# qcc4cp/qcc

Hardware: AMD Instinct MI355X
Metric: gate-applies/sec (2^30-amplitude units), QFT (higher is better)
Workload: dtype f64; 1 GPU; 30-qubit QFT complex128, 465 gates/step (qc.qft order), basis-state input, state resident in HBM, 2^30 amplitudes per GPU [BASELINE config 2]; qubits=30, fusion=1

## Files before the change

### include/qcc_hip.h

```cpp
#ifndef QCC_HIP_H_
#define QCC_HIP_H_

#include <stdint.h>

#ifdef __cplusplus
extern "C" {
#endif

typedef struct qh_state_s *qh_handle;

#define QH_OK 0
#define QH_ERR_BAD_QUBIT 1
#define QH_ERR_SAME_QUBIT 2
#define QH_ERR_BAD_DTYPE 3
#define QH_ERR_HIP 4
#define QH_ERR_ARG 5
#define QH_ERR_NOMEM 6
#define QH_ERR_NO_DEVICE 7
#define QH_ERR_NONLOCAL 8
#define QH_ERR_COMM 9

#define QH_FUSE_OFF 0
#define QH_FUSE_SWEEP 1

// ... 77 lines not shown
int qh_comm_unique_id(void *id );
int qh_comm_init(qh_handle h, int nranks, int rank, const void *id);
int qh_comm_init_custom(qh_handle h, int nranks, int rank, qh_round_fn fn, void *user);
int qh_comm_destroy(qh_handle h);
int qh_exchange_alltoall(qh_handle h, int base_bit, uint64_t chunk_amps);
int qh_exchange_pair(qh_handle h, int shard_bit, int local_bit, uint64_t chunk_amps);
int qh_exchange_loopback(qh_handle h, int local_bit, uint64_t chunk_amps);
int qh_exchange_wait(qh_handle h);
int qh_exchange_stats(qh_handle h, qh_xstats *out);
int qh_comm_allreduce_sum(qh_handle h, double *inout, int count);

int qh_norm2(qh_handle h, double *out);
int qh_amplitude(qh_handle h, uint64_t logical_index, double out[2]);
int qh_argmax(qh_handle h, uint64_t *phys_index, double *prob);
int qh_prob_bit(qh_handle h, int logical_bit, double *p1);
int qh_prob_bit_value(qh_handle h, int logical_bit, int value, double *p);
int qh_scale(qh_handle h, double re, double im);
int qh_project_bit(qh_handle h, int logical_bit, int value);
int qh_marginal(qh_handle h, int k, const int32_t *bits, double *out);
int qh_sample(qh_handle h, uint64_t count, const double *u, uint64_t *logical_out);
int qh_project_bits(qh_handle h, uint64_t mask, uint64_t value);
int qh_expect_pauli(qh_handle h, uint64_t nterms, const uint64_t *xmask, const uint64_t *zmask, double *out);

typedef struct {
  uint64_t gates_submitted;
  uint64_t kernels_launched;
  uint64_t sweeps;
  uint64_t bytes_algorithmic;
  uint64_t bytes_swept;
  uint64_t gates_noop;
} qh_stats;
int qh_get_stats(qh_handle h, qh_stats *out);
int qh_reset_stats(qh_handle h);
int qh_timer_begin(qh_handle h);
int qh_timer_end(qh_handle h, float *milliseconds);
int qh_timer_lap(qh_handle h);
int qh_timer_laps(qh_handle h, float *milliseconds, int cap, int *count);
int qh_plan_json(qh_handle h, char *buf, uint64_t cap, uint64_t *needed);

int qh_plan_export(qh_handle h, void *buf, uint64_t cap, uint64_t *needed);

int qh_plan_handlers(qh_handle h, void *buf, uint64_t cap, uint64_t *needed);

int qh_host_apply1(void *psi, const double gate[8], int nbits, int tgt,
                   int bit_width);
int qh_host_applyc(void *psi, const double gate[8], int nbits, int ctl, int tgt,
                   int bit_width);
int qh_host_release(void);

#ifdef __cplusplus
}
#endif
#endif
```

### qcc_amd/csrc/engine.hip

```cpp
#include <hip/hip_runtime.h>

#include <algorithm>
#include <chrono>
#include <cmath>
#include <cstdarg>
#include <cstddef>
#include <cstdio>
#include <cstdlib>
#include <cstring>
#include <ctime>
#include <string>
#include <vector>

#include "../../include/qcc_hip.h"
#include "kernels_gate.hip.h"
#include "kernels_dense.hip.h"
#include "kernels_mux.hip.h"
#include "kernels_measure.hip.h"
#include "kernels_expect.hip.h"
#include "planner.h"
#include "kernels_sweep.hip.h"

namespace {

// ... 306 lines not shown
        abort_comm_and_drain(h);
        return fail(QH_ERR_COMM, "%s: rank %d of %d still waiting after %.0f s (QH_COMM_TIMEOUT_MS): a peer is missing or the "
                    "ranks disagree about an exchange; the communicator was aborted, the state of this handle is undefined", what,
                    h->comm->rank, h->comm->nranks, ms * 1e-3);
      }
      struct timespec ts = {0, 50000};
      nanosleep(&ts, nullptr);
    }
  }
}
int wait_stream(qh_state_s *h, hipStream_t s, const char *what) {
  if (!watched(h)) {
    HIP_TRY(hipStreamSynchronize(s));
    return QH_OK;
  }
  return poll_until_done(h, [&] { return hipStreamQuery(s); }, what);
}
int wait_event(qh_state_s *h, hipEvent_t e, const char *what) {
  if (!watched(h)) {
    HIP_TRY(hipEventSynchronize(e));
    return QH_OK;
  }
  return poll_until_done(h, [&] { return hipEventQuery(e); }, what);
}

bool relayout_eligible(const qh_state_s *h) {
  return env_int("QH_RELAYOUT", 1) != 0 && h->owns_mem && !h->host_psi && qh::sweep_supported(h->nloc, h->bw);
}
bool relayout_wanted(const qh_state_s *h) {
  if (h->dry) return env_int("QH_RELAYOUT", 1) != 0;
  if (h->relayout >= 0) return h->relayout == 1;
  return relayout_eligible(h) && !(h->comm && h->comm->nranks > 1);
}
qh::PlanRequest plan_request(const qh_state_s *h, bool relayout) {
  return qh::PlanRequest{h->nloc, h->bw, h->shard, relayout, h->nglob > h->nloc, qh::PlanSwitches::from_env()};
}
hipError_t alloc_state_buffer(void **p, size_t bytes) {
  static const int contig = env_int("QH_ALLOC_CONTIG", -1), debug = env_int("QH_ALLOC_DEBUG", 0);
  const auto t0 = std::chrono::steady_clock::now();
  hipError_t e = hipErrorOutOfMemory;
  bool got_contig = false;
  const bool want_contig = contig < 0 ? (bytes >= (4ull << 30) && bytes <= (32ull << 30)) : (contig > 0 && bytes >= (64ull << 20));
  if (want_contig) {
    e = hipExtMallocWithFlags(p, bytes, hipDeviceMallocContiguous);
    got_contig = e == hipSuccess;
    if (!got_contig) {
      (void)hipGetLastError();
      *p = nullptr;
    }
  }
  if (!got_contig) e = hipMalloc(p, bytes);
  if (debug)
    fprintf(stderr, "[qh alloc %zu MiB %s at %p in %.1f ms]\n", bytes >> 20, got_contig ? "contiguous" : "plain", *p,
            std::chrono::duration<double, std::milli>(std::chrono::steady_clock::now() - t0).count());
  return e;
}
bool second_buffer_fits(const qh_state_s *h, size_t bytes) {
  size_t fr = 0, total = 0;
  const size_t reserve = (bytes >> 5) + (3ull << 29) + ((h->comm && h->comm->nranks > 1) ? (4ull << 30) : 0);
  return hipMemGetInfo(&fr, &total) == hipSuccess && fr > bytes + reserve;
}
bool alloc_second_buffer(qh_state_s *h) {
  if (h->d_alt) return true;
  const size_t bytes = (size_t)h->amp_bytes() << h->nloc;
  if (second_buffer_fits(h, bytes) && alloc_state_buffer(&h->d_alt, bytes) == hipSuccess)
    return true;
  (void)hipGetLastError();
  h->d_alt = nullptr;
// ... 46 lines not shown
  }
  if (borrowed) {
    if (rc) (void)hipStreamSynchronize(h->stream);
    (void)hipFree(h->d_alt);
    h->d_alt = nullptr;
  } else if (rc == QH_OK) {
    std::swap(h->d_psi, h->d_alt);
  }
  if (rc) return rc;
  for (size_t k = 0; k < loc.size(); ++k) h->perm[loc[k]] = posn[k];
  return QH_OK;
}

int flush_impl(qh_state_s *h, qh::SlabIO *split = nullptr, qh::TileMaxOut *tmax = nullptr) {
  int rc = use_device(h);
  if (rc) return rc;
  if (h->poisoned)
    return fail(QH_ERR_HIP, "the state of this handle is undefined: a sweep of an earlier flush failed after others had run; "
                            "re-initialise it (qh_init_basis / qh_init_product / qh_upload of the whole shard)");
  std::vector<qh::Arrival> *arr = (h->comm && !h->comm->arrivals.empty()) ? &h->comm->arrivals : nullptr;
  if (h->queue.empty()) {
    qh::wait_all_arrivals(arr, h->stream);
    return QH_OK;
  }
  if (h->fusion == QH_FUSE_SWEEP && qh::sweep_supported(h->nloc, h->bw)) {
    const uint64_t launched0 = h->stats.kernels_launched;
    qh::SlabIO local;
    qh::SlabIO *io = split ? split : &local;
    io->arrivals = arr;
    io->comm = h->comm;
    const bool relay = relayout_ready(h);
    void *result = h->d_psi;
    uint8_t final_pos[64];
    rc = qh::run_fused(h->queue, plan_request(h, relay), h->d_psi, h->stream, h->dry, &h->sweep, &h->stats, &g_err,
                       h->comm ? io : nullptr, h->d_alt, &result, final_pos, tmax);
    if (rc == QH_OK && relay) {
      if (result != h->d_psi) std::swap(h->d_psi, h->d_alt);
      for (int b = 0; b < h->nglob; ++b)
        if (h->perm[b] < h->nloc) h->perm[b] = final_pos[h->perm[b]];
    }
    qh::wait_all_arrivals(arr, h->stream);
    if (h->comm) h->comm->stats.sweeps_overlapped += io->sweeps_overlapped;
    if (rc != QH_OK && h->stats.kernels_launched == launched0) return rc;
    if (rc == QH_OK) rc = check_launch(h);
    if (rc != QH_OK) {
      g_err += " [sweeps of this flush may have run partially: its gates were dropped and the state is undefined until re-initialised]";
      h->poisoned = true;
    }
    h->queue.clear();
    return rc;
  }
  qh::wait_all_arrivals(arr, h->stream);
  size_t done = 0;
  for (const auto &r : h->queue) {
    rc = launch_single(h, r);
    if (rc == QH_OK) rc = check_launch(h);
    if (rc) break;
    ++done;
  }
  h->queue.erase(h->queue.begin(), h->queue.begin() + done);
  return rc;
}

int enter(qh_state_s *h) {
  if (h->dry) return fail(QH_ERR_ARG, "not on a dry (planner-only) handle");
  return flush_impl(h);
}
// ... 1352 lines not shown
      for (uint32_t u = 0; u < (1u << per_bits); ++u) a.zu[k] |= (uint16_t)((__builtin_popcount(u & zu) & 1) << u);
      a.zc[k] = z >> nom;
      const uint32_t one = (((tm.ny >> 1) ^ tm.neg) & 1u) ? 0xBFF00000u : 0x3FF00000u;
      if (tm.ny & 1u) a.cim[k] = one; else a.cre[k] = one;
    }
    const int tt = cnt <= 4 ? 4 : qh::kExpectT;
    with_real(h, [&](auto x) {
      using R = decltype(x);
      if (tt == 4) launch_expect<R, 4>(h, pair, (unsigned)nblk, a, slab);
      else launch_expect<R, qh::kExpectT>(h, pair, (unsigned)nblk, a, slab);
    });
    hipLaunchKernelGGL(qh::k_expect_fold, dim3((unsigned)cnt), dim3(256), 0, h->stream, (const double *)slab, (uint32_t)nblk, tt,
                       pair ? 2.0 : 1.0, dout + first);
    if ((rc = check_launch(h))) return rc;
    first += cnt;
    ++batches;
  }
  std::vector<double> vals(nterms);
  if ((rc = read_back(h, vals.data(), dout, (size_t)nterms * sizeof(double)))) return rc;
  for (uint64_t k = 0; k < nterms; ++k) out[terms[k].idx] = vals[k];
  h->stats.kernels_launched += batches;
  h->stats.bytes_swept += batches * ((1ull << h->nloc) * h->amp_bytes());
  return QH_OK;
}

int qh_get_stats(qh_handle h, qh_stats *out) {
  if (!h || !out) return fail(QH_ERR_ARG, "null");
  *out = h->stats;
  return QH_OK;
}
int qh_reset_stats(qh_handle h) {
  if (!h) return fail(QH_ERR_ARG, "null");
  h->stats = qh_stats{};
  return QH_OK;
}

int qh_timer_begin(qh_handle h) {
  if (!h) return fail(QH_ERR_ARG, "null handle");
  int rc = enter(h);
  if (rc) return rc;
  rc = make_events(h);
  if (rc) return rc;
  HIP_TRY(hipEventRecord(h->ev0, h->stream));
  return QH_OK;
}
int qh_timer_end(qh_handle h, float *ms) {
  if (!h || !ms) return fail(QH_ERR_ARG, "null handle or out");
  if (!h->ev0) return fail(QH_ERR_ARG, "qh_timer_end without qh_timer_begin");
  int rc = enter(h);
  if (rc) return rc;
  HIP_TRY(hipEventRecord(h->ev1, h->stream));
  if ((rc = wait_event(h, h->ev1, "qh_timer_end"))) return rc;
  HIP_TRY(hipEventElapsedTime(ms, h->ev0, h->ev1));
  return QH_OK;
}

int qh_timer_lap(qh_handle h) {
  if (!h) return fail(QH_ERR_ARG, "null handle");
  const int rc = enter(h);
  if (rc) return rc;
  if (h->laps_used == h->laps.size()) {
    hipEvent_t e = nullptr;
    HIP_TRY(hipEventCreate(&e));
    h->laps.push_back(e);
  }
  HIP_TRY(hipEventRecord(h->laps[h->laps_used++], h->stream));
// ... 718 lines not shown
```

### qcc_amd/csrc/kernels_sweep.hip.h

```cpp
#pragma once
#include <hip/hip_runtime.h>

#include <string>
#include <vector>

#include "kernels_gate.hip.h"
#include <deque>
#include <memory>

#include "planner.h"
#include "exchange.hip.h"

namespace qh {

struct SweepParams {
  const SweepOp *ops;
  const DGroup *groups;
  const OTerm *oterms;
  uint32_t nops;
  uint32_t tables_rel;
  uint32_t n_ltab_lds;
  uint32_t pad0;
  uint64_t store_delta_mask;
  uint64_t prof_buf;
// ... 292 lines not shown
      memcpy(&o->cm_reg, &g.re, 8);
      memcpy(&o->cm_thread, &g.im, 8);
    }
  if (!sp.groups.empty()) memcpy(groups_out, sp.groups.data(), sp.groups.size() * sizeof(DGroup));
  for (size_t k = 0; k < sp.groups.size(); ++k) {
    DGroup *g = groups_out + k;
    if (n_ltab_lds && (g->flags & DG_LTAB) && g->ltab_off / 64 < n_ltab_lds) g->flags |= DG_LTAB_LDS;
    bool sign_ot = !(g->flags & (DG_LTAB | DG_BITFAC)) && g->ntab == 0 && g->n_oterms > 0 && g->re == 1.0 && g->im == 0.0;
    for (uint32_t t = 0; sign_ot && t < g->n_oterms; ++t) {
      const OTerm &o = sp.oterms[g->oterm_off + t];
      sign_ot = o.re == -1.0 && o.im == 0.0;
    }
    g->flags |= group_handler_bits(*g, sp.rb, sign_ot);
  }
}

struct PlanCacheEntry {
  std::vector<GateRec> queue;
  std::string key;
  std::shared_ptr<const PlanResult> plan;
};

inline bool same_queue(const std::vector<GateRec> &a, const std::vector<GateRec> &b) {
  if (a.size() != b.size()) return false;
  for (size_t i = 0; i < a.size(); ++i)
    if (a[i].ctl_mask != b[i].ctl_mask || a[i].tgt != b[i].tgt || a[i].neg_mask != b[i].neg_mask ||
        memcmp(a[i].g, b[i].g, sizeof a[i].g) != 0)
      return false;
  return true;
}

struct SweepBuffers {
  std::deque<PlanCacheEntry> plans;
  void *d_buf = nullptr;
  size_t cap = 0;
  void *h_pinned = nullptr;
  size_t cap_host = 0;
  hipEvent_t copied = nullptr;
};

inline void free_sweep_buffers(SweepBuffers *b) {
  if (b->copied) {
    (void)hipEventSynchronize(b->copied);
    (void)hipEventDestroy(b->copied);
  }
  if (b->d_buf) (void)hipFree(b->d_buf);
  if (b->h_pinned) (void)hipHostFree(b->h_pinned);
  *b = SweepBuffers{};
}

inline bool sweep_supported(int nloc, int bw) { return (bw == 128 || bw == 64) && nloc >= kLaneBits + 2; }

template <bool WIDE> inline void sweep_block_shape(const SweepPlan &sp, int *wpb, size_t *exch_bytes) {
  const bool contiguous = sp.contiguous();
  *wpb = contiguous ? 2 : 4;
  *exch_bytes = 0;
  if (sp.nwave) {
    *wpb = 1 << sp.nwave;
    const int nr = 1 << sp.rb;
    *exch_bytes = (size_t)*wpb * std::min(8, nr / 2) * 64 * (WIDE ? 16 : 8);
  }
}

template <bool WIDE> inline int ltab_lds_count(const SweepPlan &sp) {
  constexpr int cap = 16;
  int wpb;
  size_t exch;
  sweep_block_shape<WIDE>(sp, &wpb, &exch);
  const long per_wg = 160l * 1024 * wpb / 12 - (long)exch - 512;
  const int fit = (int)std::max(0l, per_wg / 1024);
  return std::max(0, std::min(std::min(sp.n_ltab, cap), fit));
}

inline int sweep_rot(bool contiguous) { return contiguous ? 3 : 6; }

inline uint64_t sweep_tile_bits(const SweepPlan &sp) {
  uint64_t m = ((1ull << sp.lane_low) - 1) | sp.fixed_ones;
  for (int k = 0; k < sp.rb; ++k) m |= (1ull << sp.regpos[k]) | (1ull << sp.regpos_store[k]);
  for (int k = 0; k < sp.nlanehi(); ++k) m |= 1ull << sp.lanehi[k];
  for (int k = 0; k < sp.nwave; ++k) m |= 1ull << sp.wavepos[k];
  return m;
// ... 120 lines not shown
  uint64_t tile_mask = 0;
};

struct SlabIO {
  std::vector<Arrival> *arrivals = nullptr;
  bool split_last = false;
  uint64_t avoid = 0;
  int want_bits = 3;
  Comm *comm = nullptr;
  uint64_t slab_mask = 0;
  std::vector<uint64_t> slab_vals;
  std::vector<hipEvent_t> slab_done;
  bool split_done = false;
  uint64_t sweeps_overlapped = 0;
};

inline void wait_all_arrivals(std::vector<Arrival> *arr, hipStream_t stream) {
  if (!arr) return;
  for (const Arrival &a : *arr) if (a.ev) (void)hipStreamWaitEvent(stream, a.ev, 0);
  arr->clear();
}

inline int run_fused(const std::vector<GateRec> &queue, const PlanRequest &rq, void *psi, hipStream_t stream, bool dry,
                     SweepBuffers *bufs, qh_stats *stats, std::string *err, SlabIO *slab = nullptr, void *psi_alt = nullptr,
                     void **result = nullptr, uint8_t *final_pos = nullptr, TileMaxOut *tmax = nullptr) {
  const int nloc = rq.nloc, bw = rq.bw;
  const uint64_t shard = rq.shard;
  std::shared_ptr<const PlanResult> cached;
  const int rc = guard_planning(err, [&] {
    const std::string key = rq.key();
    const bool use_cache = !getenv("QH_PLAN_CACHE") || atoi(getenv("QH_PLAN_CACHE")) != 0;
    if (use_cache)
      for (auto &e : bufs->plans)
        if (e.key == key && same_queue(e.queue, queue)) { cached = e.plan; return; }
    cached = std::make_shared<const PlanResult>(plan_best(queue, rq));
    if (use_cache) {
      bufs->plans.push_front(PlanCacheEntry{queue, key, cached});
      if (bufs->plans.size() > 4) bufs->plans.pop_back();
    }
  });
  if (rc) return rc;
  const PlanResult &pr = *cached;
  const int pace = dry ? 0 : flush_pace(pr, bw == 128, nloc);
  stats->gates_noop += pr.noop_gates;
  size_t n_ops = 0, n_groups = 0, n_ot = 0, n_tab = 0;
  for (auto &sp : pr.sweeps) {
    if (popc(sp.fixed_ones) + sp.rb + sp.nlanehi() + sp.nwave > kMaxIns) {
      *err = "sweep needs more inserted bits than the tile enumeration supports";
      return QH_ERR_ARG;
    }
    n_ops += sp.ops.size() + 1;
    n_groups += sp.groups.size();
    n_ot += sp.oterms.size();
    n_tab += sp.tables.size();
  }
  const bool want_tmax = tmax && tmax->buf && !dry && !slab && !pr.sweeps.empty() && pr.sweeps.back().fixed_ones == 0 &&
                         (pr.sweeps.back().ntiles >> pr.sweeps.back().nwave) <= tmax->cap;
  if (tmax) tmax->valid = false;
  const size_t bytes_prm = pr.sweeps.size() * sizeof(SweepParams);
  const size_t bytes_ops = n_ops * sizeof(SweepOp), bytes_groups = n_groups * sizeof(DGroup),
               bytes_ot = (n_ot * sizeof(OTerm) + 15) / 16 * 16, bytes_tab = n_tab * sizeof(double);
  const size_t total = bytes_prm + bytes_ops + bytes_groups + bytes_ot + bytes_tab + 256;
  if (!dry && bufs->cap < total) {
    if (bufs->d_buf) {
      (void)hipStreamSynchronize(stream);
      (void)hipFree(bufs->d_buf);
    }
    const size_t cap = std::max<size_t>(total * 2, 1 << 20);
// ... 285 lines not shown
```

### qcc_amd/csrc/planner.h

```cpp
#pragma once
#include <sched.h>
#include <stdint.h>

#include <algorithm>
#include <atomic>
#include <cassert>
#include <cmath>
#include <cstdio>
#include <cstdlib>
#include <cstring>
#include <exception>
#include <new>
#include <string>
#include <thread>
#include <vector>

#include "../../include/qcc_hip.h"

namespace qh {

struct GateRec {
  uint64_t ctl_mask;
  int tgt;
  double g[8];
  uint64_t neg_mask = 0;
  uint8_t ghost = 0, variant = 0;
  uint8_t force_dense = 0;
};

inline bool is_diag(const double g[8]) {
  return g[2] == 0.0 && g[3] == 0.0 && g[4] == 0.0 && g[5] == 0.0;
}
inline bool is_one(double re, double im) { return re == 1.0 && im == 0.0; }
inline bool plan_diag(const double g[8], int tgt) {
  return is_diag(g) && (tgt < 0 || !(g[0] == 0.0 && g[1] == 0.0));
}
inline bool plan_diag(const GateRec &r) { return !r.force_dense && plan_diag(r.g, r.tgt); }

constexpr int kLaneBits = 6;
constexpr int kLaneLow = 3;
constexpr int kLaneHi = 3;
constexpr int kMaxLaneHiBit = 27;
constexpr int kMaxRegBits = 6;
inline int max_reg_bits(int bw) { return bw == 128 ? 5 : 6; }
// ... 5 lines not shown
enum : uint32_t { OP_DENSE_REG = 0, OP_DENSE_LANE = 1, OP_DIAG = 2,
                  OP_LSWAP = 3,
                  OP_WSWAP = 4 };
enum : uint32_t { OPF_DEFER_C = 1, OPF_USE_C = 2, OPF_REAL = 4,
                  OPF_BFLY = 8, OPF_BFLY_SHIFT = 4,
                  OPF_LANE_DPP = 128, OPF_SWAP_RI = 256,
                  OPF_GHOST = 1024,
                  OPF_ROT_P = 2048, OPF_ROT_M = 4096 };

inline bool env_flag(const char *name, bool dflt) {
  const char *e = getenv(name);
  return e ? atoi(e) != 0 : dflt;
}

inline int env_int(const char *name, int dflt) {
  const char *e = getenv(name);
  return e ? atoi(e) : dflt;
}

struct PlanSwitches {
  bool wave_pinned = false;
  int wave_bits = 1;
  bool split_lanes = true;
  int max_rb = kMaxRegBits;
  bool bfly = true, propagate_x = true, defer_diag = true, rot_fuse = true;
  int lane_valu = 1, seats = 1;
  bool search = true, search_wb2 = true;
  bool steps_pinned = false; uint64_t steps = 0;
  int streams = 0;
  int only_wb = -1, pick = -1;
  int tiles_wb = 0;
  std::vector<std::vector<int>> tiles;
  bool threads = true, log = false, dag = false, verbose = false;

  static PlanSwitches from_env() {
    PlanSwitches w;
    if (const char *e = getenv("QH_WAVE_BITS")) { w.wave_pinned = true; w.wave_bits = std::max(0, std::min(kMaxWaveBits, atoi(e))); }
    w.split_lanes = env_flag("QH_SPLIT_LANES", true);
    w.max_rb = std::max(2, std::min(kMaxRegBits, env_int("QH_SWEEP_RB", kMaxRegBits)));
    w.bfly = env_flag("QH_BFLY", true), w.propagate_x = env_flag("QH_PROPAGATE_X", true);
    w.defer_diag = env_flag("QH_DEFER_DIAG", true), w.rot_fuse = env_flag("QH_ROT_FUSE", true);
    w.lane_valu = env_int("QH_LANE_VALU", 1), w.seats = env_int("QH_SEATS", 1);
    w.search = env_flag("QH_PLAN_SEARCH", true), w.search_wb2 = env_flag("QH_PLAN_SEARCH_WB2", true);
    if (const char *e = getenv("QH_PLAN_SEARCH_STEPS")) { w.steps_pinned = true; w.steps = strtoull(e, nullptr, 10); }
    if (const char *e = getenv("QH_PLAN_SEARCH_STREAMS")) w.streams = std::max(1, std::min(8, atoi(e)));
    w.only_wb = env_int("QH_PLAN_ONLY_WB", -1), w.pick = env_int("QH_PLAN_SEARCH_PICK", -1);
    if (const char *e = getenv("QH_PLAN_TILES")) {
      w.tiles.emplace_back();
      w.tiles_wb = atoi(e);
      const char *p = strchr(e, ':');
      for (p = p ? p + 1 : e; *p; ++p) {
        if (*p == ';') w.tiles.emplace_back();
        else if (*p != ',') { char *end = nullptr; w.tiles.back().push_back((int)strtol(p, &end, 10)); if (end == p) break; p = end - 1; }
      }
    }
    w.threads = env_flag("QH_PLAN_SEARCH_THREADS", true), w.log = env_flag("QH_PLAN_SEARCH_LOG", false);
    w.dag = env_flag("QH_PLAN_DAG", false), w.verbose = env_flag("QH_PLAN_VERBOSE", false);
    return w;
  }
  std::string key() const {
    char b[192];
    snprintf(b, sizeof b, "%d,%d;%d;%d;%d%d%d%d;%d;%d;%d%d;%d,%llu;%d;%d;%d;%d:", wave_pinned, wave_bits, split_lanes, max_rb, bfly,
             propagate_x, defer_diag, rot_fuse, lane_valu, seats, search, search_wb2, steps_pinned, (unsigned long long)steps, streams,
             only_wb, pick, tiles_wb);
    std::string s = b;
    for (const auto &t : tiles) {
      s += ';';
      for (int v : t) s += std::to_string(v) + ',';
    }
    return s;
  }
};

struct PlanRequest {
  int nloc, bw;
  uint64_t shard;
  bool relayout;
  bool keep_ghosts;
  PlanSwitches sw;
  std::string key() const {
    return std::to_string(nloc) + "," + std::to_string(bw) + "," + std::to_string(shard) + "," + std::to_string(relayout) +
           std::to_string(keep_ghosts) + ":" + sw.key();
  }
};

inline int butterfly_variant(const double *g) {
  const double cr = g[0], ci = g[1];
  if (cr == 0.0 && ci == 0.0) return -1;
  auto eq = [&](int k, double r, double i) { return g[2 * k] == r && g[2 * k + 1] == i; };
  if (eq(1, cr, ci) && eq(2, cr, ci) && eq(3, -cr, -ci)) return 0;
  if (eq(1, -cr, -ci) && eq(2, cr, ci) && eq(3, cr, ci)) return 1;
  if (eq(1, cr, ci) && eq(2, -cr, -ci) && eq(3, cr, ci)) return 2;
  if (eq(1, ci, -cr) && eq(2, ci, -cr) && eq(3, cr, ci)) return 3;
  if (eq(1, -ci, cr) && eq(2, -ci, cr) && eq(3, cr, ci)) return 4;
  return -1;
}

struct OTerm {
  uint64_t mask;
  double re, im;
};
constexpr uint32_t DG_LTAB = 1u;
constexpr uint32_t DG_LTAB_LDS = 2u;
constexpr uint32_t DG_BITFAC = 8u;
constexpr int kBitFacs = 4;
inline int bitfac_others(int rb, int j, int out[kBitFacs]) {
  int n = 0;
  for (int b = 0; b < rb && n < kBitFacs; ++b) if (b != j) out[n++] = b;
  return n;
}
struct DGroup {
  uint32_t lane_mask, reg_mask;
// ... 23 lines not shown
  int nlanehi() const { return kLaneBits - lane_low; }
  int seat[kLaneBits] = {0, 1, 2, 3, 4, 5};
  int seat_store[kLaneBits] = {0, 1, 2, 3, 4, 5};
  int seat_dest[kLaneBits] = {0, 1, 2, 3, 4, 5};
  bool contiguous() const {
    for (int k = 0; k < nlanehi(); ++k) if (lanehi[k] != lane_low + k) return false;
    return true;
  }
  int nwave = 0;
  int wavepos[kMaxWaveBits] = {0};
  uint64_t fixed_ones = 0;
  uint64_t ntiles = 0;
  bool relayout = false;
  uint8_t dest_pos[64] = {0};
  int wavepos_store[kMaxWaveBits] = {0};
  int reg_dest[kMaxRegBits] = {6, 7, 8, 9, 10, 11};
  int wave_dest[kMaxWaveBits] = {11, 12};
  std::vector<SweepOp> ops;
  std::vector<DGroup> groups;
  std::vector<OTerm> oterms;
  std::vector<double> tables;
  std::vector<double> ltabs;
  int n_ltab = 0;
  uint64_t gates = 0;
  uint64_t alg_bytes = 0;
  uint64_t swept_bytes = 0;
};

struct PlanResult {
  std::vector<SweepPlan> sweeps;
  uint64_t noop_gates = 0;
  bool moved = false;
  uint8_t final_pos[64];
  PlanResult() { for (int p = 0; p < 64; ++p) final_pos[p] = (uint8_t)p; }
};

inline int popc(uint64_t x) { return __builtin_popcountll(x); }

inline uint64_t gate_alg_bytes(const GateRec &r, int nloc, uint64_t amp_bytes) {
  const uint64_t lm = (nloc >= 64) ? ~0ull : ((1ull << nloc) - 1);
  const int nc = popc(r.ctl_mask & lm);
  const bool diag = is_diag(r.g);
  uint64_t touched = 1ull << (nloc - nc);
  if (diag && r.tgt < nloc && is_one(r.g[0], r.g[1])) touched >>= 1;
  return touched * amp_bytes * 2;
}

constexpr int kMaxUnitSegs = 8;
inline int unit_segments(const SweepPlan &sp, int nloc, uint64_t *masks, int *shifts) {
  uint64_t tile = 0;
  for (int i = 0; i < kLaneBits; ++i) tile |= 1ull << sp.seat_store[i];
  for (int k = 0; k < sp.rb; ++k) tile |= 1ull << sp.regpos_store[k];
  for (int k = 0; k < sp.nwave; ++k) tile |= 1ull << sp.wavepos_store[k];
  const int tilebits = popc(tile);
  int nseg = 0, i = 0, last_shift = 1 << 20;
  for (int p = 0; p < nloc; ++p) {
    if ((tile >> p) & 1ull) continue;
    const int shift = ((int)sp.dest_pos[p] - tilebits) - i;
    if (shift != last_shift) {
      ++nseg;
      last_shift = shift;
      if (masks && nseg <= kMaxUnitSegs) { masks[nseg - 1] = 0; shifts[nseg - 1] = shift; }
    }
    if (masks && nseg <= kMaxUnitSegs) masks[nseg - 1] |= 1ull << i;
    ++i;
  }
// ... 143 lines not shown
      if (last_dense[tb] >= 0) ps.push_back(last_dense[tb]);
      for (int u : need[tb]) ps.push_back(u);
      for (uint64_t t = r.diag_bits; t; t &= t - 1) if (last_dense[__builtin_ctzll(t)] >= 0) ps.push_back(last_dense[__builtin_ctzll(t)]);
      std::sort(ps.begin(), ps.end());
      ps.erase(std::unique(ps.begin(), ps.end()), ps.end());
      for (int u : ps) { (*succ)[u].push_back(v); (*pred)[v].push_back(u); }
      need[tb].clear();
      last_dense[tb] = v;
      for (uint64_t t = r.diag_bits; t; t &= t - 1) need[__builtin_ctzll(t)].push_back(v);
    }
  }
  std::string dag_json(const std::vector<GateRec> &queue) {
    std::vector<GateRec> pending;
    std::vector<uint64_t> alg;
    uint64_t noops = 0;
    prepare(queue, &pending, &alg, &noops);
    std::vector<PassRec> rec0;
    int back[64];
    uint64_t movable = 0;
    canonical_records(pending, &rec0, back, &movable);
    std::vector<int> node_bit;
    std::vector<std::vector<int>> succ, pred;
    build_dag(rec0, &node_bit, &succ, &pred);
    std::string o = "{\"line_bits\":" + std::to_string(lane_low_) + ",\"cap_per_wave_bits\":[" + std::to_string(lane_hi_ + rb_cap_) + "," +
                    std::to_string(lane_hi_ + rb_cap_ + 1) + "," + std::to_string(lane_hi_ + rb_cap_ + 2) + "],\"target_bit\":[";
    for (size_t g = 0; g < node_bit.size(); ++g) o += (g ? "," : "") + std::to_string(back[node_bit[g]]);
    o += "],\"edges\":[";
    bool first = true;
    for (size_t u = 0; u < succ.size(); ++u)
      for (int v : succ[u]) { o += (first ? "[" : ",[") + std::to_string(u) + "," + std::to_string(v) + "]"; first = false; }
    return o + "]}";
  }
  bool search_levels(const std::vector<GateRec> &queue, size_t K, uint64_t change_budget, uint64_t stream,
                     std::vector<std::vector<int>> *tiles_out, uint64_t *changes_used = nullptr) {
    if (changes_used) *changes_used = 0;
    if (K < 2 || K > 8) return false;
    std::vector<GateRec> pending;
    std::vector<uint64_t> alg;
    uint64_t noops = 0;
    prepare(queue, &pending, &alg, &noops);
    std::vector<PassRec> rec0;
    int back[64];
    uint64_t movable = 0;
    canonical_records(pending, &rec0, back, &movable);
    const uint64_t always = (1ull << lane_low_) - 1;
    const int cap = lane_hi_ + rb_cap_ + max_wave_;
    if ((size_t)popc(movable) > K * (size_t)cap) return false;
    std::vector<int> node_bit;
    std::vector<std::vector<int>> succ, pred;
    build_dag(rec0, &node_bit, &succ, &pred);
    const int ng = (int)node_bit.size();
    if (!ng) return false;
    std::vector<int> depth(ng, 0);
    int maxd = 0;
    for (int u = 0; u < ng; ++u) for (int v : succ[u]) { depth[v] = std::max(depth[v], depth[u] + 1); maxd = std::max(maxd, depth[v]); }
    std::vector<int> chain[64];
    for (int g = 0; g < ng; ++g) chain[node_bit[g]].push_back(g);
    std::vector<int8_t> L(ng);
    int occ[64][8], ntile[8];
    uint64_t changes = 0;
    auto set_level = [&](int g, int to) {
      const int q = node_bit[g], from = L[g];
      ++changes;
      if (!((always >> q) & 1)) {
        if (--occ[q][from] == 0) --ntile[from];
        if (occ[q][to]++ == 0) ++ntile[to];
      }
// ... 17 lines not shown
    };
    std::vector<int> stk;
    std::vector<std::pair<int, int8_t>> undo;
    auto move = [&](int g, bool down) {
      const int to = L[g] + (down ? -1 : 1);
      if (to < 0 || to >= (int)K) return false;
      stk.assign(1, g);
      undo.emplace_back(g, L[g]);
      set_level(g, to);
      while (!stk.empty()) {
        const int u = stk.back();
        stk.pop_back();
        for (int v : down ? pred[u] : succ[u])
          if (down ? L[v] > to : L[v] < to) { undo.emplace_back(v, L[v]); set_level(v, to); stk.push_back(v); }
      }
      return true;
    };
    auto revert = [&]() { for (size_t i = undo.size(); i-- > 0;) set_level(undo[i].first, undo[i].second); undo.clear(); };
    uint64_t rng = 0x9e3779b97f4a7c15ull * (2 * stream + 1);
    auto rnd = [&](uint32_t n) { rng ^= rng << 13; rng ^= rng >> 7; rng ^= rng << 17; return (uint32_t)((rng >> 11) % n); };
    constexpr long kRestart = 1500;
    constexpr int kTenure = 7;
    std::vector<long> tabu((size_t)ng * 2);
    std::vector<int> cands;
    bool found = false;
    for (long walk = 0; !found; ++walk) {
      init();
      std::fill(tabu.begin(), tabu.end(), -1);
      int over = 0, best_over = 0;
      long best_key = cost(&best_over);
      over = best_over;
      for (long it = 0; it < kRestart && over > 0; ++it) {
        if (++changes > change_budget) goto out;
        if (walk == 0 && it == 400 && best_over > 4) goto out;
        cands.clear();
        for (size_t s = 0; s < K; ++s) {
          if (ntile[s] <= cap) continue;
          for (uint64_t t = movable; t; t &= t - 1) {
            const int q = __builtin_ctzll(t);
            if (!occ[q][s]) continue;
            int first = -1, last = -1;
            for (int g : chain[q]) if (L[g] == (int8_t)s) { if (first < 0) first = g; last = g; }
            cands.push_back(first * 2);
            cands.push_back(last * 2 + 1);
          }
        }
        long bk = 1L << 60;
        int bm = -1, ties = 0;
        for (int m : cands) {
          undo.clear();
          if (!move(m >> 1, m & 1)) continue;
          int o = 0;
          const long k = cost(&o);
          revert();
          if (tabu[m] > it && !(o < best_over)) continue;
          if (k < bk) { bk = k; bm = m; ties = 1; }
          else if (k == bk && rnd((uint32_t)++ties) == 0) bm = m;
        }
        if (bm < 0) continue;
        undo.clear();
        move(bm >> 1, bm & 1);
        const long k = cost(&over);
        for (const auto &u : undo) tabu[(size_t)u.first * 2 + ((bm & 1) ? 0 : 1)] = it + kTenure + (long)rnd(kTenure);
        if (k < best_key) { best_key = k; best_over = over; }
      }
      found = over == 0;
// ... 1318 lines not shown
  uint64_t dense_bits = 0;
  for (const GateRec &q : queue) if (q.tgt >= 0 && q.tgt < nloc && !plan_diag(q.g, q.tgt)) dense_bits |= 1ull << q.tgt;
  const int lane_low = bw == 128 ? 3 : 4;
  const int cap0 = (kLaneBits - lane_low) + std::min({sw.max_rb, max_reg_bits(bw), nloc - kLaneBits});
  if (best_n >= 3 && sw.search) {
    const double sweep_us = 2.0 * (double)(bw == 128 ? 16 : 8) * (double)(1ull << nloc) / 5.5e6;
    const uint64_t budget = sw.steps_pinned ? sw.steps : std::min<uint64_t>((uint64_t)(sweep_us * 640.0), 5000000);
    struct Task {
      int wb;
      size_t K;
      uint64_t stream, used = 0;
      bool ok = false, planned = false;
      double ms = 0;
      PlanResult pr;
      std::exception_ptr failed;
    };
    std::vector<Task> tasks;
    const size_t nmovable = (size_t)popc(dense_bits >> lane_low);
    std::vector<std::pair<int, size_t>> shapes;
    for (int wb : {1, 2, 0}) {
      if (budget < 5000) break;
      if (wb != best_wb && (wb == 0 || far_of[wb] || n_of[wb] == 0 || best_n < 4 || (wb == 2 && !sw.search_wb2))) continue;
      if (only_wb >= 0 && wb != only_wb) continue;
      const size_t cap = (size_t)(cap0 + wb), greedy = n_of[wb];
      const size_t kmin = std::max<size_t>({2, (nmovable + cap - 1) / cap, greedy > 3 ? greedy - 3 : 0});
      for (size_t K = kmin; K + 1 <= greedy && K <= best_n && K <= 8; ++K) shapes.emplace_back(wb, K);
    }
    int streams = 6;
    if (const unsigned hw = usable_cpus(); hw && !keep_ghosts && !shapes.empty())
      streams = std::max(1, std::min(6, (int)(hw / shapes.size())));
    if (sw.streams) streams = sw.streams;
    for (const auto &sh : shapes)
      for (int s = 0; s < streams; ++s) { tasks.emplace_back(); tasks.back().wb = sh.first; tasks.back().K = sh.second; tasks.back().stream = (uint64_t)(s + 1); }
    auto run = [&](Task &t) {
      const size_t i = (size_t)(&t - &tasks[0]);
      try {
        std::vector<std::vector<int>> tiles;
        t.ok = Planner(rq, t.wb).search_levels(queue, t.K, budget, t.stream, &tiles, &t.used);
        if (!t.ok) return;
        Planner forced(rq, t.wb);
        forced.set_tiles(tiles);
        t.pr = forced.plan(queue);
        t.planned = t.pr.sweeps.size() <= t.K && !plan_has_far_tile(t.pr);
      } catch (...) { t.failed = std::current_exception(); return; }
      if (t.planned) t.ms = keep_ghosts ? 1000.0 * (double)t.pr.sweeps.size() + 1e-3 * (double)(i + 1) : plan_predicted_ms(t.pr, nloc, bw);
    };
    std::atomic<size_t> next{0};
    auto drain = [&] { for (size_t i; (i = next++) < tasks.size(); ) run(tasks[i]); };
    std::vector<std::thread> pool;
    const size_t workers = sw.threads ? std::min<size_t>(tasks.size(), usable_cpus()) : 0;
    try { while (pool.size() < workers) pool.emplace_back(drain); } catch (...) {}
    PlanResult greedy_plan;
    std::exception_ptr greedy_failed;
    try { greedy_plan = chosen.plan(queue); } catch (...) { greedy_failed = std::current_exception(); next = tasks.size(); }
    drain();
    for (std::thread &x : pool) x.join();
    if (greedy_failed) std::rethrow_exception(greedy_failed);
    const Task *win = nullptr;
    double best_ms = keep_ghosts ? 1000.0 * (double)greedy_plan.sweeps.size() : plan_predicted_ms(greedy_plan, nloc, bw);
    for (const Task &t : tasks)
      if (t.planned && t.pr.sweeps.size() <= greedy_plan.sweeps.size() && t.ms < best_ms) { win = &t; best_ms = t.ms; }
    if (sw.pick >= 0) {
      if ((size_t)sw.pick < tasks.size() && tasks[sw.pick].planned) win = &tasks[sw.pick];
    }
    if (sw.log) {
      for (const Task &t : tasks)
        fprintf(stderr, "[qh plan search]   task %d: wave bits %d K=%zu stream %llu: %s after %llu label changes%s\n", (int)(&t - &tasks[0]), t.wb, t.K, (unsigned long long)t.stream,
                t.failed ? "FAILED (exception)" : t.ok ? "found" : "not found", (unsigned long long)t.used,
                t.planned ? (", " + std::to_string(t.pr.sweeps.size()) + " sweeps, predicted " + std::to_string(t.ms) + " ms").c_str() : "");
      fprintf(stderr, "[qh plan search] greedy: %d wave bit(s), %zu sweeps, predicted %.2f ms; chosen: %s (%zu tasks, budget %llu label changes each)\n", best_wb,
              greedy_plan.sweeps.size(), plan_predicted_ms(greedy_plan, nloc, bw),
              win ? (std::to_string(win->pr.sweeps.size()) + " sweeps with " + std::to_string(win->wb) + " wave bit(s), predicted " + std::to_string(win->ms) + " ms").c_str() : "greedy",
              tasks.size(), (unsigned long long)budget);
    }
    if (keep_ghosts)
      for (const Task &t : tasks) if (t.failed) std::rethrow_exception(t.failed);
    if (win) return win->pr;
    return greedy_plan;
  }
  return chosen.plan(queue);
}

template <class F> int guard_planning(std::string *err, F &&f) {
  try { f(); } catch (const std::bad_alloc &) { *err = "planning: out of host memory"; return QH_ERR_NOMEM; }
  catch (const std::exception &e) { *err = std::string("planning: ") + e.what(); return QH_ERR_ARG; }
  return QH_OK;
}

inline std::string plan_to_json(const std::vector<GateRec> &queue, const PlanRequest &rq) {
  if (rq.nloc < kLaneBits + 2) return "{\"sweeps\":[],\"note\":\"state too small for sweeps\"}";
  PlanResult pr = plan_best(queue, rq);
  std::string s = "{\"noop_gates\":" + std::to_string(pr.noop_gates);
  if (rq.sw.dag)
    s += ",\"dag\":" + Planner(rq, 1).dag_json(queue);
  s += ",\"sweeps\":[";
  char buf[384];
  for (size_t i = 0; i < pr.sweeps.size(); ++i) {
    const SweepPlan &sp = pr.sweeps[i];
    int nd = 0, ndiag = 0, nbf = 0;
    int nswap = 0, ndpp = 0;
    for (auto &o : sp.ops) {
      if (o.kind == OP_LSWAP || o.kind == OP_WSWAP) { nswap++; continue; }
      (o.kind == OP_DIAG ? ndiag : nd)++;
      if (o.flags & OPF_BFLY) nbf++;
      if (o.flags & OPF_LANE_DPP) ndpp++;
    }
    std::string rp = "[";
    for (int k = 0; k < sp.rb; ++k) rp += (k ? "," : "") + std::to_string(sp.regpos[k]);
    rp += "],\"lanehi\":[";
    for (int k = 0; k < sp.nlanehi(); ++k) rp += (k ? "," : "") + std::to_string(sp.lanehi[k]);
// ... 35 lines not shown
```

### qcc_amd/device.py

```python
import ctypes

import numpy as np

from qcc_amd import gates as _gates
from qcc_amd import native

_dp = ctypes.POINTER(ctypes.c_double)
MAX_MARGINAL_BITS = 16


def _g8(gate):
  g = _gates.as8(gate)
  return g, g.ctypes.data_as(_dp)


def merge_factors(factors, table_bits=12, max_factors=32):
  out = []
  for n, x in factors:
    n = int(n)
    if n == 0:
      continue
    is_int = isinstance(x, (int, np.integer))
    if out:
      pn, px = out[-1]
# ... 290 lines not shown
    z = np.ascontiguousarray([int(v) for v in zmasks], dtype=np.uint64)
    if x.size != z.size:
      raise ValueError(f'expect_pauli: {x.size} x masks, {z.size} z masks')
    out = np.zeros(x.size, dtype=np.float64)
    u64p = ctypes.POINTER(ctypes.c_uint64)
    native.check(self.lib.qh_expect_pauli(self.h, int(x.size), x.ctypes.data_as(u64p), z.ctypes.data_as(u64p),
                                          out.ctypes.data_as(_dp)))
    return out

  def project_bits(self, mask, value):
    native.check(self.lib.qh_project_bits(self.h, int(mask), int(value)))

  def phys_to_logical(self, i):
    o = ctypes.c_uint64()
    native.check(self.lib.qh_phys_to_logical(self.h, int(i), ctypes.byref(o)))
    return o.value

  def logical_to_phys(self, i):
    o = ctypes.c_uint64()
    native.check(self.lib.qh_logical_to_phys(self.h, int(i), ctypes.byref(o)))
    return o.value

  def remap_swap(self, a, b):
    native.check(self.lib.qh_remap_swap(self.h, int(a), int(b)))

  def amplitude(self, logical_index):
    out = (ctypes.c_double * 2)()
    native.check(self.lib.qh_amplitude(self.h, int(logical_index), out))
    return self.dtype(complex(out[0], out[1]))

  def stats(self):
    s = native.QhStats()
    native.check(self.lib.qh_get_stats(self.h, ctypes.byref(s)))
    return s.as_dict()

  def reset_stats(self):
    native.check(self.lib.qh_reset_stats(self.h))

  def timer_begin(self):
    native.check(self.lib.qh_timer_begin(self.h))

  def timer_end(self):
    ms = ctypes.c_float()
    native.check(self.lib.qh_timer_end(self.h, ctypes.byref(ms)))
    return ms.value

  def timer_lap(self):
    native.check(self.lib.qh_timer_lap(self.h))

  def timer_laps(self, cap=4096):
    buf = (ctypes.c_float * cap)()
    n = ctypes.c_int(0)
    native.check(self.lib.qh_timer_laps(self.h, buf, cap, ctypes.byref(n)))
    return [float(buf[k]) for k in range(min(n.value, cap))]

  def plan_json(self):
    need = ctypes.c_uint64()
    native.check(self.lib.qh_plan_json(self.h, None, 0, ctypes.byref(need)))
    buf = ctypes.create_string_buffer(need.value)
    native.check(self.lib.qh_plan_json(self.h, buf, need.value, None))
    return buf.value.decode()


NO_CTL = -(2 ** 31)
```

### qcc_amd/native.py

```python
import ctypes
import os
import subprocess

PKG = os.path.dirname(os.path.abspath(__file__))
ROOT = os.path.dirname(PKG)
LIB_PATH = os.environ.get('QCC_HIP_LIB') or os.path.join(PKG, 'libqcc_hip.so')
SOURCES = [os.path.join(PKG, 'csrc', f) for f in
           ('engine.hip', 'kernels_gate.hip.h', 'kernels_dense.hip.h', 'kernels_mux.hip.h', 'kernels_measure.hip.h', 'kernels_expect.hip.h', 'kernels_sweep.hip.h', 'planner.h', 'exchange.hip.h',
            'sweep_island_rb2.inc', 'sweep_island_rb3.inc', 'sweep_island_rb4.inc',
            'sweep_island_rb5.inc', 'sweep_island_f32_rb2.inc', 'sweep_island_f32_rb3.inc',
            'sweep_island_f32_rb4.inc', 'sweep_island_f32_rb5.inc', 'sweep_island_f32_rb6.inc', 'sweep_handlers.inc',
            'libq_facade.cc')]
HEADERS = [os.path.join(ROOT, 'include', 'libq.h')]
HEADER = os.path.join(ROOT, 'include', 'qcc_hip.h')

QH_OK = 0
QH_ERR_BAD_QUBIT, QH_ERR_SAME_QUBIT, QH_ERR_BAD_DTYPE, QH_ERR_HIP = 1, 2, 3, 4
QH_ERR_ARG, QH_ERR_NOMEM, QH_ERR_NO_DEVICE, QH_ERR_NONLOCAL, QH_ERR_COMM = 5, 6, 7, 8, 9
QH_FUSE_OFF, QH_FUSE_SWEEP = 0, 1

_u64, _i32, _vp, _dp = ctypes.c_uint64, ctypes.c_int, ctypes.c_void_p, ctypes.POINTER(ctypes.c_double)


class QhStats(ctypes.Structure):
  _fields_ = [('gates_submitted', _u64), ('kernels_launched', _u64), ('sweeps', _u64),
              ('bytes_algorithmic', _u64), ('bytes_swept', _u64), ('gates_noop', _u64)]

  def as_dict(self):
    return {k: int(getattr(self, k)) for k, _ in self._fields_}


SIGNATURES = {
    'qh_last_error': (ctypes.c_char_p, []),
    'qh_version': (_i32, []),
    'qh_device_count': (_i32, [ctypes.POINTER(_i32)]),
    'qh_create': (_i32, [_i32, _i32, _i32, ctypes.POINTER(_vp)]),
    'qh_attach': (_i32, [_i32, _i32, _i32, _vp, _vp, ctypes.POINTER(_vp)]),
    'qh_create_dry': (_i32, [_i32, _i32, ctypes.POINTER(_vp)]),
    'qh_create_host_mapped': (_i32, [_i32, _i32, _i32, ctypes.POINTER(_vp)]),
    'qh_host_ptr': (_i32, [_vp, ctypes.POINTER(_vp)]),
    'qh_destroy': (_i32, [_vp]),
    'qh_set_shard': (_i32, [_vp, _i32, _u64]),
    'qh_device_ptr': (_i32, [_vp, ctypes.POINTER(_vp)]),
    'qh_stream': (_i32, [_vp, ctypes.POINTER(_vp)]),
    'qh_nbits': (_i32, [_vp, ctypes.POINTER(_i32), ctypes.POINTER(_i32)]),
    'qh_init_basis': (_i32, [_vp, _u64]),
    'qh_init_product': (_i32, [_vp, _i32, ctypes.POINTER(_i32), ctypes.POINTER(_vp), ctypes.POINTER(_u64)]),
    'qh_upload': (_i32, [_vp, _vp, _u64, _u64]),
    'qh_download': (_i32, [_vp, _vp, _u64, _u64]),
    'qh_apply1': (_i32, [_vp, _i32, _dp]),
    'qh_applyc': (_i32, [_vp, _i32, _i32, _dp]),
    'qh_apply_bits': (_i32, [_vp, _u64, _i32, _dp]),
    'qh_apply_matrix': (_i32, [_vp, _i32, ctypes.POINTER(ctypes.c_int32), _u64, _dp]),
    'qh_apply_mux': (_i32, [_vp, _i32, ctypes.POINTER(ctypes.c_int32), _i32, _dp]),
    'qh_apply_diag': (_i32, [_vp, _i32, ctypes.POINTER(ctypes.c_int32), _dp]),
    'qh_set_fusion': (_i32, [_vp, _i32]),
    'qh_set_relayout': (_i32, [_vp, _i32, ctypes.POINTER(_i32)]),
    'qh_apply_stream': (_i32, [_vp, _u64, ctypes.POINTER(ctypes.c_int32), _dp]),
    'qh_flush': (_i32, [_vp]),
    'qh_sync': (_i32, [_vp]),
    'qh_pending_gates': (_i32, [_vp, ctypes.POINTER(_u64)]),
    'qh_discard_pending': (_i32, [_vp]),
    'qh_remap_swap': (_i32, [_vp, _i32, _i32]),
    'qh_get_bitmap': (_i32, [_vp, ctypes.POINTER(ctypes.c_int32)]),
    'qh_phys_to_logical': (_i32, [_vp, _u64, ctypes.POINTER(_u64)]),
    'qh_logical_to_phys': (_i32, [_vp, _u64, ctypes.POINTER(_u64)]),
    'qh_norm2': (_i32, [_vp, _dp]),
    'qh_amplitude': (_i32, [_vp, _u64, _dp]),
    'qh_argmax': (_i32, [_vp, ctypes.POINTER(_u64), _dp]),
    'qh_prob_bit': (_i32, [_vp, _i32, _dp]),
    'qh_prob_bit_value': (_i32, [_vp, _i32, _i32, _dp]),
    'qh_scale': (_i32, [_vp, ctypes.c_double, ctypes.c_double]),
    'qh_project_bit': (_i32, [_vp, _i32, _i32]),
    'qh_marginal': (_i32, [_vp, _i32, ctypes.POINTER(ctypes.c_int32), _dp]),
    'qh_sample': (_i32, [_vp, _u64, _dp, ctypes.POINTER(ctypes.c_uint64)]),
    'qh_project_bits': (_i32, [_vp, _u64, _u64]),
    'qh_expect_pauli': (_i32, [_vp, _u64, ctypes.POINTER(_u64), ctypes.POINTER(_u64), _dp]),
    'qh_get_stats': (_i32, [_vp, ctypes.POINTER(QhStats)]),
    'qh_reset_stats': (_i32, [_vp]),
    'qh_timer_begin': (_i32, [_vp]),
    'qh_timer_end': (_i32, [_vp, ctypes.POINTER(ctypes.c_float)]),
    'qh_timer_lap': (_i32, [_vp]),
    'qh_timer_laps': (_i32, [_vp, ctypes.POINTER(ctypes.c_float), _i32, ctypes.POINTER(_i32)]),
    'qh_plan_json': (_i32, [_vp, ctypes.c_char_p, _u64, ctypes.POINTER(_u64)]),
    'qh_plan_export': (_i32, [_vp, _vp, _u64, ctypes.POINTER(_u64)]),
    'qh_plan_handlers': (_i32, [_vp, _vp, _u64, ctypes.POINTER(_u64)]),
    'qh_host_apply1': (_i32, [_vp, _dp, _i32, _i32, _i32]),
    'qh_host_applyc': (_i32, [_vp, _dp, _i32, _i32, _i32, _i32]),
    'qh_host_release': (_i32, []),
}


class QhXStats(ctypes.Structure):
  _fields_ = [('exchanges', _u64), ('rounds', _u64), ('bytes_sent', _u64), ('slabs', _u64),
              ('sweeps_overlapped', _u64), ('span_ms', ctypes.c_double), ('rounds_packed', _u64),
              ('geometry_checks', _u64), ('comm_ranks', ctypes.c_uint32), ('comm_rank', ctypes.c_uint32)]

  def as_dict(self):
    return {k: getattr(self, k) for k, _ in self._fields_}


class QhXGeom(ctypes.Structure):
  _fields_ = [('signature', _u64), ('slab_mask', _u64), ('block_bits', _u64), ('rounds_per_slab', _u64), ('staging_bytes', _u64),
              ('slabs', ctypes.c_uint32), ('chunk_bits', ctypes.c_uint32), ('packed', ctypes.c_uint32), ('peers', ctypes.c_uint32),
              ('sweeps_before', ctypes.c_uint32), ('last_sweep_split', ctypes.c_uint32)]

  def as_dict(self):
    return {k: int(getattr(self, k)) for k, _ in self._fields_}


ROUND_FN = ctypes.CFUNCTYPE(ctypes.c_int, _vp, ctypes.c_int, ctypes.POINTER(ctypes.c_int), ctypes.POINTER(_vp),
                            ctypes.POINTER(_vp), _u64)
# ... 74 lines not shown
```

Before: 28300 gate-applies/s.

## Use quick cancellable plan search when GPU stream is idle, upgrade cached plans later

When the stream is idle at flush time, planning time sits on the critical path, so the planner runs a reduced-budget search with cancellation, takes the smallest-K tile plan that succeeds, and skips predicted-cost ranking. Cached quick plans are replaced by a full search on a later flush when the GPU is busy and planning can overlap execution. Plan statistics counters and an API to read them are added. The trade-off is that an exposed flush may run a somewhat worse sweep schedule.

Result: no change. 28250 gate-applies/s (-0.2%).

```diff
diff --git a/include/qcc_hip.h b/include/qcc_hip.h
--- a/include/qcc_hip.h
+++ b/include/qcc_hip.h
@@ -133,6 +133,13 @@
 } qh_stats;
 int qh_get_stats(qh_handle h, qh_stats *out);
 int qh_reset_stats(qh_handle h);
+typedef struct {
+  uint64_t plans_full;
+  uint64_t plans_quick;
+  uint64_t cache_hits;
+  uint64_t cache_upgrades;
+} qh_plan_stats;
+int qh_get_plan_stats(qh_handle h, qh_plan_stats *out);
 int qh_timer_begin(qh_handle h);
 int qh_timer_end(qh_handle h, float *milliseconds);
 int qh_timer_lap(qh_handle h);
diff --git a/qcc_amd/csrc/engine.hip b/qcc_amd/csrc/engine.hip
--- a/qcc_amd/csrc/engine.hip
+++ b/qcc_amd/csrc/engine.hip
@@ -362,8 +362,16 @@
   if (h->relayout >= 0) return h->relayout == 1;
   return relayout_eligible(h) && !(h->comm && h->comm->nranks > 1);
 }
-qh::PlanRequest plan_request(const qh_state_s *h, bool relayout) {
-  return qh::PlanRequest{h->nloc, h->bw, h->shard, relayout, h->nglob > h->nloc, qh::PlanSwitches::from_env()};
+qh::PlanRequest plan_request(const qh_state_s *h, bool relayout, bool idle = false) {
+  qh::PlanRequest rq{h->nloc, h->bw, h->shard, relayout, h->nglob > h->nloc, qh::PlanSwitches::from_env()};
+  rq.exposed = !rq.keep_ghosts && (rq.sw.exposed >= 0 ? rq.sw.exposed == 1 : idle);
+  return rq;
+}
+bool stream_idle(const qh_state_s *h) {
+  if (h->dry || (h->comm && !h->comm->arrivals.empty())) return false;
+  const bool idle = hipStreamQuery(h->stream) == hipSuccess;
+  if (!idle) (void)hipGetLastError();
+  return idle;
 }
 hipError_t alloc_state_buffer(void **p, size_t bytes) {
   static const int contig = env_int("QH_ALLOC_CONTIG", -1), debug = env_int("QH_ALLOC_DEBUG", 0);
@@ -476,7 +484,7 @@
     const bool relay = relayout_ready(h);
     void *result = h->d_psi;
     uint8_t final_pos[64];
-    rc = qh::run_fused(h->queue, plan_request(h, relay), h->d_psi, h->stream, h->dry, &h->sweep, &h->stats, &g_err,
+    rc = qh::run_fused(h->queue, plan_request(h, relay, stream_idle(h)), h->d_psi, h->stream, h->dry, &h->sweep, &h->stats, &g_err,
                        h->comm ? io : nullptr, h->d_alt, &result, final_pos, tmax);
     if (rc == QH_OK && relay) {
       if (result != h->d_psi) std::swap(h->d_psi, h->d_alt);
@@ -1895,6 +1903,12 @@
 int qh_reset_stats(qh_handle h) {
   if (!h) return fail(QH_ERR_ARG, "null");
   h->stats = qh_stats{};
+  h->sweep.pstats = qh_plan_stats{};
+  return QH_OK;
+}
+int qh_get_plan_stats(qh_handle h, qh_plan_stats *out) {
+  if (!h || !out) return fail(QH_ERR_ARG, "null");
+  *out = h->sweep.pstats;
   return QH_OK;
 }
 
diff --git a/qcc_amd/csrc/kernels_sweep.hip.h b/qcc_amd/csrc/kernels_sweep.hip.h
--- a/qcc_amd/csrc/kernels_sweep.hip.h
+++ b/qcc_amd/csrc/kernels_sweep.hip.h
@@ -348,6 +348,7 @@
 
 struct SweepBuffers {
   std::deque<PlanCacheEntry> plans;
+  qh_plan_stats pstats{};
   void *d_buf = nullptr;
   size_t cap = 0;
   void *h_pinned = nullptr;
@@ -356,6 +357,7 @@
 };
 
 inline void free_sweep_buffers(SweepBuffers *b) {
+  const qh_plan_stats keep = b->pstats;
   if (b->copied) {
     (void)hipEventSynchronize(b->copied);
     (void)hipEventDestroy(b->copied);
@@ -363,6 +365,7 @@
   if (b->d_buf) (void)hipFree(b->d_buf);
   if (b->h_pinned) (void)hipHostFree(b->h_pinned);
   *b = SweepBuffers{};
+  b->pstats = keep;
 }
 
 inline bool sweep_supported(int nloc, int bw) { return (bw == 128 || bw == 64) && nloc >= kLaneBits + 2; }
@@ -549,8 +552,19 @@
     const bool use_cache = !getenv("QH_PLAN_CACHE") || atoi(getenv("QH_PLAN_CACHE")) != 0;
     if (use_cache)
       for (auto &e : bufs->plans)
-        if (e.key == key && same_queue(e.queue, queue)) { cached = e.plan; return; }
+        if (e.key == key && same_queue(e.queue, queue)) {
+          if (e.plan->quick && !rq.exposed) {
+            e.plan = std::make_shared<const PlanResult>(plan_best(queue, rq));
+            bufs->pstats.cache_upgrades++;
+            bufs->pstats.plans_full++;
+          } else {
+            bufs->pstats.cache_hits++;
+          }
+          cached = e.plan;
+          return;
+        }
     cached = std::make_shared<const PlanResult>(plan_best(queue, rq));
+    (cached->quick ? bufs->pstats.plans_quick : bufs->pstats.plans_full)++;
     if (use_cache) {
       bufs->plans.push_front(PlanCacheEntry{queue, key, cached});
       if (bufs->plans.size() > 4) bufs->plans.pop_back();
diff --git a/qcc_amd/csrc/planner.h b/qcc_amd/csrc/planner.h
--- a/qcc_amd/csrc/planner.h
+++ b/qcc_amd/csrc/planner.h
@@ -10,6 +10,7 @@
 #include <cstdlib>
 #include <cstring>
 #include <exception>
+#include <memory>
 #include <new>
 #include <string>
 #include <thread>
@@ -81,6 +82,7 @@
   int tiles_wb = 0;
   std::vector<std::vector<int>> tiles;
   bool threads = true, log = false, dag = false, verbose = false;
+  int exposed = -1;
 
   static PlanSwitches from_env() {
     PlanSwitches w;
@@ -105,6 +107,7 @@
     }
     w.threads = env_flag("QH_PLAN_SEARCH_THREADS", true), w.log = env_flag("QH_PLAN_SEARCH_LOG", false);
     w.dag = env_flag("QH_PLAN_DAG", false), w.verbose = env_flag("QH_PLAN_VERBOSE", false);
+    if (const char *e = getenv("QH_PLAN_EXPOSED")) w.exposed = (*e == 'a' || *e == 'A' || !*e) ? -1 : (atoi(e) != 0 ? 1 : 0);
     return w;
   }
   std::string key() const {
@@ -127,6 +130,7 @@
   bool relayout;
   bool keep_ghosts;
   PlanSwitches sw;
+  bool exposed = false;
   std::string key() const {
     return std::to_string(nloc) + "," + std::to_string(bw) + "," + std::to_string(shard) + "," + std::to_string(relayout) +
            std::to_string(keep_ghosts) + ":" + sw.key();
@@ -216,6 +220,7 @@
   uint64_t noop_gates = 0;
   bool moved = false;
   uint8_t final_pos[64];
+  bool quick = false;
   PlanResult() { for (int p = 0; p < 64; ++p) final_pos[p] = (uint8_t)p; }
 };
 
@@ -425,7 +430,8 @@
     return o + "]}";
   }
   bool search_levels(const std::vector<GateRec> &queue, size_t K, uint64_t change_budget, uint64_t stream,
-                     std::vector<std::vector<int>> *tiles_out, uint64_t *changes_used = nullptr) {
+                     std::vector<std::vector<int>> *tiles_out, uint64_t *changes_used = nullptr,
+                     const std::atomic<uint32_t> *cancel = nullptr) {
     if (changes_used) *changes_used = 0;
     if (K < 2 || K > 8) return false;
     std::vector<GateRec> pending;
@@ -509,6 +515,7 @@
       over = best_over;
       for (long it = 0; it < kRestart && over > 0; ++it) {
         if (++changes > change_budget) goto out;
+        if (cancel && cancel->load(std::memory_order_relaxed)) goto out;
         if (walk == 0 && it == 400 && best_over > 4) goto out;
         cands.clear();
         for (size_t s = 0; s < K; ++s) {
@@ -1893,17 +1900,30 @@
     if (sw.streams) streams = sw.streams;
     for (const auto &sh : shapes)
       for (int s = 0; s < streams; ++s) { tasks.emplace_back(); tasks.back().wb = sh.first; tasks.back().K = sh.second; tasks.back().stream = (uint64_t)(s + 1); }
+    const bool quick = rq.exposed;
+    constexpr uint64_t kQuickGiveUpNum = 3, kQuickGiveUpDen = 8;
+    const uint64_t quick_num = std::min<uint64_t>(kQuickGiveUpDen, (kQuickGiveUpNum * 6 + (uint64_t)streams - 1) / (uint64_t)streams);
+    const uint64_t task_budget = quick ? budget / kQuickGiveUpDen * quick_num : budget;
+    std::unique_ptr<std::atomic<uint32_t>[]> cancel(new std::atomic<uint32_t>[tasks.size() + 1]);
+    for (size_t i = 0; i <= tasks.size(); ++i) cancel[i].store(0, std::memory_order_relaxed);
+    auto cancelled = [&](size_t i) { return quick && cancel[i].load(std::memory_order_relaxed) != 0; };
     auto run = [&](Task &t) {
       const size_t i = (size_t)(&t - &tasks[0]);
       try {
+        if (cancelled(i)) return;
         std::vector<std::vector<int>> tiles;
-        t.ok = Planner(rq, t.wb).search_levels(queue, t.K, budget, t.stream, &tiles, &t.used);
-        if (!t.ok) return;
+        t.ok = Planner(rq, t.wb).search_levels(queue, t.K, task_budget, t.stream, &tiles, &t.used, quick ? &cancel[i] : nullptr);
+        if (!t.ok || cancelled(i)) return;
         Planner forced(rq, t.wb);
         forced.set_tiles(tiles);
         t.pr = forced.plan(queue);
         t.planned = t.pr.sweeps.size() <= t.K && !plan_has_far_tile(t.pr);
       } catch (...) { t.failed = std::current_exception(); return; }
+      if (quick) {
+        if (t.planned)
+          for (size_t j = i + 1; j < tasks.size(); ++j) if (tasks[j].K >= t.K) cancel[j].store(1, std::memory_order_relaxed);
+        return;
+      }
       if (t.planned) t.ms = keep_ghosts ? 1000.0 * (double)t.pr.sweeps.size() + 1e-3 * (double)(i + 1) : plan_predicted_ms(t.pr, nloc, bw);
     };
     std::atomic<size_t> next{0};
@@ -1919,8 +1939,10 @@
     if (greedy_failed) std::rethrow_exception(greedy_failed);
     const Task *win = nullptr;
     double best_ms = keep_ghosts ? 1000.0 * (double)greedy_plan.sweeps.size() : plan_predicted_ms(greedy_plan, nloc, bw);
-    for (const Task &t : tasks)
-      if (t.planned && t.pr.sweeps.size() <= greedy_plan.sweeps.size() && t.ms < best_ms) { win = &t; best_ms = t.ms; }
+    for (const Task &t : tasks) {
+      if (!t.planned || t.pr.sweeps.size() > greedy_plan.sweeps.size()) continue;
+      if (quick ? (!win || t.K < win->K) : t.ms < best_ms) { win = &t; best_ms = t.ms; }
+    }
     if (sw.pick >= 0) {
       if ((size_t)sw.pick < tasks.size() && tasks[sw.pick].planned) win = &tasks[sw.pick];
     }
@@ -1936,7 +1958,8 @@
     }
     if (keep_ghosts)
       for (const Task &t : tasks) if (t.failed) std::rethrow_exception(t.failed);
-    if (win) return win->pr;
+    if (win) greedy_plan = win->pr;
+    greedy_plan.quick = quick && !tasks.empty();
     return greedy_plan;
   }
   return chosen.plan(queue);
diff --git a/qcc_amd/device.py b/qcc_amd/device.py
--- a/qcc_amd/device.py
+++ b/qcc_amd/device.py
@@ -346,6 +346,11 @@
   def stats(self):
     s = native.QhStats()
     native.check(self.lib.qh_get_stats(self.h, ctypes.byref(s)))
+    return dict(s.as_dict(), **self.plan_stats())
+
+  def plan_stats(self):
+    s = native.QhPlanStats()
+    native.check(self.lib.qh_get_plan_stats(self.h, ctypes.byref(s)))
     return s.as_dict()
 
   def reset_stats(self):
diff --git a/qcc_amd/native.py b/qcc_amd/native.py
--- a/qcc_amd/native.py
+++ b/qcc_amd/native.py
@@ -25,6 +25,13 @@
 class QhStats(ctypes.Structure):
   _fields_ = [('gates_submitted', _u64), ('kernels_launched', _u64), ('sweeps', _u64),
               ('bytes_algorithmic', _u64), ('bytes_swept', _u64), ('gates_noop', _u64)]
+
+  def as_dict(self):
+    return {k: int(getattr(self, k)) for k, _ in self._fields_}
+
+
+class QhPlanStats(ctypes.Structure):
+  _fields_ = [('plans_full', _u64), ('plans_quick', _u64), ('cache_hits', _u64), ('cache_upgrades', _u64)]
 
   def as_dict(self):
     return {k: int(getattr(self, k)) for k, _ in self._fields_}
@@ -78,6 +85,7 @@
     'qh_expect_pauli': (_i32, [_vp, _u64, ctypes.POINTER(_u64), ctypes.POINTER(_u64), _dp]),
     'qh_get_stats': (_i32, [_vp, ctypes.POINTER(QhStats)]),
     'qh_reset_stats': (_i32, [_vp]),
+    'qh_get_plan_stats': (_i32, [_vp, ctypes.POINTER(QhPlanStats)]),
     'qh_timer_begin': (_i32, [_vp]),
     'qh_timer_end': (_i32, [_vp, ctypes.POINTER(ctypes.c_float)]),
     'qh_timer_lap': (_i32, [_vp]),
```
